# hasnainfarid/Custom_Gymnasium_Environments

Measured on AMD Instinct MI355X. Metric: env steps/sec (whole node) at 1M parallel envs; achieved HBM GB/s vs peak, higher is better.
Workload: dtype i8; 1 GPU; snake_1m: SnakeEnv 10x10, 1,048,576 parallel envs per GPU, random actions, fused auto-reset; envs_per_gpu=1048576, autoreset=SameStep, parallelism=env-sharded x1, no data-path collective

## Files before the change

custom_gymnasium_environments_amd/csrc/snake.hip:

```cpp
#include <cstdlib>
#include <cstring>
#include <vector>

#include "cge_device.hpp"
#include "cge_host.hpp"
#include "snake_place.hpp"

#ifndef CGE_SNAKE_FINCOPY
#define CGE_SNAKE_FINCOPY 1
#endif
namespace cge {
namespace snake {

constexpr int bitlen(int n) {
    int k = 0;
    while (n) { ++k; n >>= 1; }
    return k;
}

enum : uint32_t { F_NEEDS_RESET = 1u, F_BOARD_FULL = 2u, F_FOOD_VALID = 4u };

template <int G>
struct Lay {
    static constexpr int CELLS = G * G;
    static constexpr int OCCW = (CELLS + 31) / 32;
    static constexpr int SRW = (2 * (CELLS - 1) + 31) / 32;
    static constexpr bool TIGHT = (G == 10);
    static constexpr int HOT_SH = 15;
    static constexpr int HOT_DIRS = (2 * 32 - HOT_SH) / 2, COLD0_DIRS = 64;
    static constexpr int NW = TIGHT ? 12 : OCCW + SRW + 4;
    static constexpr int COLS = (NW + 3) / 4;
    static constexpr bool PACKED = CELLS % 4 == 0;
    static constexpr int OBS_DW = (CELLS + 3) / 4;
    static constexpr int KBITS = bitlen(G);
    static constexpr int BLOCK = (CELLS <= 144) ? 256 : 64;
    static_assert(G >= 4 && G <= 30, "center start needs G >= 4 (and a 10x10-style 3 cell margin is not assumed); 64 rows of G*G bytes + the digit rings fit 64 KB of LDS up to 30");
    static constexpr int MAX_STEPS_LIMIT = TIGHT ? 4095 : 65535;
    static constexpr uint32_t MAX_EPISODES = TIGHT ? 0xFFFFu : 0xFFFFFFFFu;
    static_assert(CELLS <= 1023, "cell index is packed in 10 bits");
    static_assert(!TIGHT || (SRW == 7 && OCCW == 4), "hot / cold split below is written for 10x10");
};

__host__ __device__ __forceinline__ int dir_delta(uint32_t d, int g) { return d == 0 ? -g : d == 1 ? 1 : d == 2 ? g : -1; }

template <int G>
struct Env {
    using L = Lay<G>;
    uint32_t occ[L::OCCW];
    uint32_t sr[L::SRW];
    uint32_t head, tail, len, food, dir, steps, score, flags, episodes, mt_pos, mt_pretw, dq_left;

    __device__ __forceinline__ void load(const uint4 *__restrict__ state, int64_t n, int64_t i) {
        uint32_t raw[L::COLS * 4];
        if constexpr (L::TIGHT) {
            const uint4 h = state[i];
            raw[0] = h.x; raw[1] = h.y; raw[2] = h.z; raw[3] = h.w;
            const uint32_t moves = ((h.x >> 7) & 127u) - 1u;
            uint4 c0 = make_uint4(0, 0, 0, 0), c1 = make_uint4(0, 0, 0, 0);
            if (moves > (uint32_t)L::HOT_DIRS) c0 = state[n + i];
            if (moves > (uint32_t)(L::HOT_DIRS + L::COLD0_DIRS)) c1 = state[2 * n + i];
            raw[4] = c0.x; raw[5] = c0.y; raw[6] = c0.z; raw[7] = c0.w;
            raw[8] = c1.x; raw[9] = c1.y; raw[10] = c1.z; raw[11] = c1.w;
        } else {
#pragma unroll
            for (int c = 0; c < L::COLS; ++c) {
                uint4 v = state[(int64_t)c * n + i];
                raw[4 * c] = v.x; raw[4 * c + 1] = v.y; raw[4 * c + 2] = v.z; raw[4 * c + 3] = v.w;
            }
        }
        unpack(raw);
    }
    __device__ __forceinline__ void store(uint4 *__restrict__ state, int64_t n, int64_t i) const {
        uint32_t raw[L::COLS * 4];
        pack(raw);
        if constexpr (L::TIGHT) {
            state[i] = make_uint4(raw[0], raw[1], raw[2], raw[3]);
            if (len - 1u > (uint32_t)L::HOT_DIRS) state[n + i] = make_uint4(raw[4], raw[5], raw[6], raw[7]);
            if (len - 1u > (uint32_t)(L::HOT_DIRS + L::COLD0_DIRS)) state[2 * n + i] = make_uint4(raw[8], raw[9], raw[10], raw[11]);
        } else {
#pragma unroll
            for (int c = 0; c < L::COLS; ++c)
                state[(int64_t)c * n + i] = make_uint4(raw[4 * c], raw[4 * c + 1], raw[4 * c + 2], raw[4 * c + 3]);
        }
    }
    __host__ __device__ __forceinline__ void unpack(const uint32_t *raw) {
        if constexpr (L::TIGHT) {
            const uint32_t w0 = raw[0], w1 = raw[1], w2 = raw[2];
            head = w0 & 127u; len = (w0 >> 7) & 127u; food = (w0 >> 14) & 127u; dir = (w0 >> 21) & 3u; flags = (w0 >> 23) & 7u;
            score = (w0 >> 26) | (((w1 >> 23) & 1u) << 6);
            steps = w1 & 0xFFFu; mt_pos = (w1 >> 12) & 1023u; mt_pretw = (w1 & (1u << 22)) ? (uint32_t)MT_N : 0u;
            episodes = (w1 >> 24) | ((w2 & 0xFFu) << 8);
            dq_left = (w2 >> 8) & 127u;
#pragma unroll
            for (int k = 0; k < L::SRW; ++k) sr[k] = (raw[2 + k] >> L::HOT_SH) | (raw[3 + k] << (32 - L::HOT_SH));
            mask_history();
            rebuild_occupancy();
        } else {
#pragma unroll
            for (int k = 0; k < L::OCCW; ++k) occ[k] = raw[k];
#pragma unroll
            for (int k = 0; k < L::SRW; ++k) sr[k] = raw[L::OCCW + k];
            const uint32_t m0 = raw[L::OCCW + L::SRW], m1 = raw[L::OCCW + L::SRW + 1], m3 = raw[L::OCCW + L::SRW + 3];
            head = m0 & 1023u; tail = (m0 >> 10) & 1023u; food = (m0 >> 20) & 1023u; dir = m0 >> 30;
            steps = m1 & 0xffffu; score = (m1 >> 16) & 1023u; flags = m1 >> 26;
            episodes = raw[L::OCCW + L::SRW + 2];
            mt_pos = m3 & 1023u; mt_pretw = (m3 & 1024u) ? (uint32_t)MT_N : 0u; len = (m3 >> 11) & 1023u; dq_left = (m3 >> 24) & 127u;
        }
    }
    __host__ __device__ __forceinline__ void pack(uint32_t *raw) const {
        if constexpr (L::TIGHT) {
            const uint32_t ep = episodes < L::MAX_EPISODES ? episodes : L::MAX_EPISODES;
            raw[0] = head | (len << 7) | (food << 14) | (dir << 21) | (flags << 23) | ((score & 63u) << 26);
            raw[1] = steps | (mt_pos << 12) | (mt_pretw ? (1u << 22) : 0u) | (((score >> 6) & 1u) << 23) | ((ep & 0xFFu) << 24);
            raw[2] = (ep >> 8) | (dq_left << 8) | (sr[0] << L::HOT_SH);
#pragma unroll
            for (int k = 1; k < L::SRW; ++k) raw[2 + k] = (sr[k - 1] >> (32 - L::HOT_SH)) | (sr[k] << L::HOT_SH);
            raw[2 + L::SRW] = sr[L::SRW - 1] >> (32 - L::HOT_SH);
#pragma unroll
            for (int k = 3 + L::SRW; k < 12; ++k) raw[k] = 0;
        } else {
#pragma unroll
            for (int k = 0; k < L::OCCW; ++k) raw[k] = occ[k];
#pragma unroll
            for (int k = 0; k < L::SRW; ++k) raw[L::OCCW + k] = sr[k];
            raw[L::OCCW + L::SRW] = head | (tail << 10) | (food << 20) | (dir << 30);
            raw[L::OCCW + L::SRW + 1] = steps | (score << 16) | (flags << 26);
            raw[L::OCCW + L::SRW + 2] = episodes;
            raw[L::OCCW + L::SRW + 3] = mt_pos | (mt_pretw ? 1024u : 0u) | (len << 11) | (dq_left << 24);
#pragma unroll
            for (int k = L::NW; k < L::COLS * 4; ++k) raw[k] = 0;
        }
    }
    __host__ __device__ __forceinline__ void mask_history() {
        const uint32_t bits = len == 0u ? 0u : 2u * (len - 1u);
#pragma unroll
        for (int k = 0; k < L::SRW; ++k) {
            const uint32_t lo = 32u * k;
            sr[k] = bits >= lo + 32u ? sr[k] : (bits > lo ? (sr[k] & ((1u << (bits - lo)) - 1u)) : 0u);
        }
    }
    __host__ __device__ __forceinline__ void rebuild_occupancy() {
#pragma unroll
        for (int k = 0; k < L::OCCW; ++k) occ[k] = 0;
        uint32_t cell = head;
        or_word(occ, cell >> 5, 1u << (cell & 31u));
        const uint32_t moves = len == 0u ? 0u : (len <= (uint32_t)L::CELLS ? len - 1u : (uint32_t)L::CELLS - 1u);
        uint64_t q = (uint64_t)sr[0] | ((uint64_t)sr[1] << 32);
        const uint32_t n1 = moves < 32u ? moves : 32u;
        for (uint32_t k = 0; k < n1; ++k) {
            cell = (uint32_t)((int)cell - dir_delta((uint32_t)q & 3u, G));
            q >>= 2;
            or_word(occ, cell >> 5, 1u << (cell & 31u));
        }
        for (uint32_t k = 32u; k < moves; ++k) {
            const uint32_t d = (sel(sr, k >> 4) >> ((k & 15u) * 2u)) & 3u;
            cell = (uint32_t)((int)cell - dir_delta(d, G));
            or_word(occ, cell >> 5, 1u << (cell & 31u));
        }
        tail = cell;
    }

    __host__ __device__ __forceinline__ uint32_t occupied(uint32_t cell) const {
        if constexpr (L::OCCW == 4) {
            const uint64_t lo = (uint64_t)occ[0] | ((uint64_t)occ[1] << 32), hi = (uint64_t)occ[2] | ((uint64_t)occ[3] << 32);
            return (uint32_t)(((cell < 64u ? lo : hi) >> (cell & 63u)) & 1ull);
        } else {
            return (sel(occ, cell >> 5) >> (cell & 31u)) & 1u;
        }
    }
    __host__ __device__ __forceinline__ uint32_t length() const { return len; }

    __device__ __forceinline__ bool can_place_food() {
        if (len >= (uint32_t)L::CELLS) {
            flags = (flags | F_BOARD_FULL) & ~F_FOOD_VALID;
            return false;
        }
        return true;
    }

    __device__ __forceinline__ void reset_body() {
#pragma unroll
        for (int k = 0; k < L::OCCW; ++k) occ[k] = 0;
#pragma unroll
        for (int k = 0; k < L::SRW; ++k) sr[k] = 0;
        constexpr uint32_t center = (G / 2) * G + (G / 2);
        head = tail = center;
        len = 1;
        occ[center >> 5] |= 1u << (center & 31u);
        dir = 1;
        score = 0;
        steps = 0;
        flags &= ~F_NEEDS_RESET;
    }

    __device__ __forceinline__ bool move(uint32_t action, uint32_t max_steps, float &reward, bool &ate, bool short_wave) {
        ate = false;
        const int d = (int)action - (int)dir;
        if (d != 2 && d != -2) dir = action;
        const uint32_t hr = head / G, hc = head - hr * G;
        int nr = (int)hr, nc = (int)hc;
        if (dir == 0) nr -= 1; else if (dir == 1) nc += 1; else if (dir == 2) nr += 1; else nc -= 1;
        const bool wall = (unsigned)nr >= (unsigned)G || (unsigned)nc >= (unsigned)G;
        const uint32_t ncell = wall ? head : (uint32_t)(nr * G + nc);
        if (wall || occupied(ncell)) {
            reward = -10.0f;
            return true;
        }
        if (!short_wave) {
#pragma unroll
            for (int k = L::SRW - 1; k > 0; --k) sr[k] = (sr[k] << 2) | (sr[k - 1] >> 30);
        }
        sr[0] = (sr[0] << 2) | dir;
        or_word(occ, ncell >> 5, 1u << (ncell & 31u));
        head = ncell;
        reward = 0.0f;
        if ((flags & F_FOOD_VALID) && ncell == food) {
            score += 1;
            len += 1;
            reward = 10.0f;
            ate = true;
        } else {
            const uint32_t p = 2u * (len - 1u);
            uint32_t td;
            if (short_wave) {
                td = (sr[0] >> p) & 3u;
                sr[0] &= ~(3u << p);
            } else {
                td = (sel(sr, p >> 5) >> (p & 31u)) & 3u;
                andnot_word(sr, p >> 5, 3u << (p & 31u));
            }
            andnot_word(occ, tail >> 5, 1u << (tail & 31u));
            tail = (uint32_t)((int)tail + dir_delta(td, G));
        }
        steps += 1;
        return steps >= max_steps;
    }

    __device__ __forceinline__ void write_obs_body(uint32_t *row) const {
#pragma unroll
        for (int j = 0; j < L::OBS_DW; ++j) {
            const uint32_t b = (occ[(4 * j) >> 5] >> ((4 * j) & 31)) & 0xFu;
            row[j] = (b * 0x00204081u) & 0x01010101u;
        }
    }
    __device__ __forceinline__ void write_obs_food(uint32_t *row) const {
        if (flags & F_FOOD_VALID) reinterpret_cast<int8_t *>(row)[food] = 2;
    }
};

struct Params {
    uint4 *state;
    uint4 *dq;
    uint32_t *mt;
    int64_t n, env0;
    const int32_t *actions;
    const uint8_t *mask;
    int8_t *obs;
    float *reward;
    uint8_t *terminated, *truncated;
    int8_t *final_obs;
    FinalSeg fin;
    int32_t mode, max_steps, k_steps;
    uint32_t dq_topup;
    uint64_t a_seed;
    int64_t t0, obs_step_stride;
    float *reward_sum;
    int32_t *done_count;
    double *ep_ret;
    int32_t *ep_len;
    unsigned long long *err_count;
};

__device__ __forceinline__ uint32_t shfl_u32(uint32_t v, uint32_t src) { return (uint32_t)__shfl((int)v, (int)src, 64); }

template <int G>
struct DigitQ {
    static constexpr int DB = Lay<G>::KBITS <= 4 ? 4 : 8;
    static constexpr int PER = 32 / DB;
    static constexpr int SLOTS = 64;
    static constexpr int QDW = SLOTS / PER;
    static constexpr int COLS = QDW / 4;
    static constexpr int QROW = QDW + 1;
    static constexpr uint32_t DMASK = (1u << DB) - 1u;
    static constexpr uint32_t ALL_COLS = (1u << COLS) - 1u;
};

template <int G>
struct DqCtx {
    uint32_t *wave_q;
    uint32_t stride;
    uint32_t *blk;
    uint4 *dq;
    int64_t n, i;
    uint32_t loaded;
    bool dirty;

    __device__ __forceinline__ uint32_t *my_row() const { return wave_q + (threadIdx.x & 63u) * stride; }
    __device__ __forceinline__ void issue_all(uint4 (&v)[DigitQ<G>::COLS]) const {
#pragma unroll
        for (int c = 0; c < DigitQ<G>::COLS; ++c) v[c] = dq[(int64_t)c * n + i];
    }
    __device__ __forceinline__ void park_all(const uint4 (&v)[DigitQ<G>::COLS]) {
        uint32_t *row = my_row();
#pragma unroll
        for (int c = 0; c < DigitQ<G>::COLS; ++c) { row[4 * c] = v[c].x; row[4 * c + 1] = v[c].y; row[4 * c + 2] = v[c].z; row[4 * c + 3] = v[c].w; }
        loaded = DigitQ<G>::ALL_COLS;
    }
    __device__ __forceinline__ void load_pair(bool want, uint32_t c0, uint32_t c1) {
        if (want && ((~loaded >> c0) & 1u || (~loaded >> c1) & 1u)) {
            uint32_t *row = my_row();
            const uint4 v0 = dq[(int64_t)c0 * n + i], v1 = dq[(int64_t)c1 * n + i];
            row[4 * c0] = v0.x; row[4 * c0 + 1] = v0.y; row[4 * c0 + 2] = v0.z; row[4 * c0 + 3] = v0.w;
            row[4 * c1] = v1.x; row[4 * c1 + 1] = v1.y; row[4 * c1 + 2] = v1.z; row[4 * c1 + 3] = v1.w;
            loaded |= (1u << c0) | (1u << c1);
        }
    }
    __device__ __forceinline__ void write_back() {
        using Q = DigitQ<G>;
        if (!dirty) return;
        const uint32_t *row = my_row();
#pragma unroll
        for (int c = 0; c < Q::COLS; ++c) dq[(int64_t)c * n + i] = make_uint4(row[4 * c], row[4 * c + 1], row[4 * c + 2], row[4 * c + 3]);
        dirty = false;
    }
};

template <int G, int RG = 2>
__device__ __forceinline__ void dq_refill(Env<G> &e, DqCtx<G> &q, unsigned long long want) {
    using L = Lay<G>;
    using Q = DigitQ<G>;
    const uint32_t lane = threadIdx.x & 63u;
    const uint32_t plo = (uint32_t)reinterpret_cast<uintptr_t>(q.blk), phi = (uint32_t)(reinterpret_cast<uintptr_t>(q.blk) >> 32);
#pragma unroll 1
    while (want) {
        int r[RG];
        bool has[RG];
        uint32_t pos[RG], pretw[RG], left[RG], fill[RG], k[RG], a[RG], b[RG], c[RG];
        uint32_t *ob[RG];
#pragma unroll
        for (int g = 0; g < RG; ++g) {
            has[g] = want != 0ull;
            r[g] = has[g] ? (int)__builtin_ctzll(want) : r[0];
            want = has[g] ? (want & (want - 1ull)) : 0ull;
            uint32_t p = lane_u32(e.mt_pos, r[g]) & 1023u, lf = lane_u32(e.dq_left, r[g]) & 127u, pt = lane_u32(e.mt_pretw, r[g]);
            p = p < (uint32_t)MT_N ? p : (uint32_t)MT_N;
            lf = lf < (uint32_t)Q::SLOTS ? lf : (uint32_t)Q::SLOTS;
            if (p == (uint32_t)MT_N && lf == 0u) { p = 0u; pt = 0u; }
            const uint32_t room = (uint32_t)Q::SLOTS - lf, rest = (uint32_t)MT_N - p;
            pos[g] = p; pretw[g] = pt; left[g] = lf; fill[g] = room < rest ? room : rest;
            const uint32_t j = (lane - p) & 63u;
            const uint32_t kk = j < fill[g] ? p + j : (p < (uint32_t)MT_N ? p : 0u);
            const uint32_t km = kk + MT_M >= (uint32_t)MT_N ? kk + MT_M - MT_N : kk + MT_M;
            k[g] = kk;
            ob[g] = lane_ptr(plo, phi, r[g]);
            a[g] = ob[g][kk]; b[g] = ob[g][kk + 1]; c[g] = ob[g][km];
        }
#pragma unroll
        for (int g = 0; g < RG; ++g) {
            if (!has[g]) continue;
            const bool active = ((lane - pos[g]) & 63u) < fill[g];
            const bool ready = k[g] < pretw[g];
            const uint32_t y = ready ? a[g] : mt_twist(a[g], b[g], c[g]);
            if (active && !ready) mt_store(ob[g], k[g], y);
            const uint32_t sh = (lane % Q::PER) * Q::DB;
            uint32_t x = active ? (mt_temper(y) >> (32 - L::KBITS)) << sh : 0u;
            uint32_t m = active ? Q::DMASK << sh : 0u;
            x |= shfl_u32(x, lane ^ 1u); m |= shfl_u32(m, lane ^ 1u);
            x |= shfl_u32(x, lane ^ 2u); m |= shfl_u32(m, lane ^ 2u);
            if (Q::PER == 8) { x |= shfl_u32(x, lane ^ 4u); m |= shfl_u32(m, lane ^ 4u); }
            uint32_t *row = q.wave_q + (uint32_t)r[g] * q.stride;
            if (lane % Q::PER == 0u && m) row[lane / Q::PER] = (row[lane / Q::PER] & ~m) | x;
            if (lane == (uint32_t)r[g]) {
                e.mt_pos = pos[g] + fill[g];
                e.mt_pretw = pretw[g];
                e.dq_left = left[g] + fill[g];
                q.dirty = true;
                q.loaded = Q::ALL_COLS;
            }
        }
    }
}

template <int G>
__device__ __forceinline__ bool dq_can_fill(const Env<G> &e) {
    return e.dq_left < (uint32_t)DigitQ<G>::SLOTS && !(e.mt_pos >= (uint32_t)MT_N && e.dq_left > 0u);
}

template <int G, bool FETCH>
__device__ __forceinline__ void dq_place_food(Env<G> &e, DqCtx<G> &q, bool need) {
    using L = Lay<G>;
    using Q = DigitQ<G>;
    const uint32_t *myq = q.my_row();
    bool pending = need;
    uint32_t phase = 0, row = 0;
#pragma unroll 1
    while (__ballot(pending)) {
        if (FETCH) {
            const uint32_t head = (e.mt_pos - e.dq_left) & 63u, d0 = head / Q::PER, d1 = (d0 + 1u) & (uint32_t)(Q::QDW - 1);
            q.load_pair(pending && e.dq_left != 0u, d0 >> 2, d1 >> 2);
        }
        const unsigned long long dry = __ballot(pending && e.dq_left < (uint32_t)Q::PER && dq_can_fill<G>(e));
// ... 280 lines not shown
        const uint32_t fin_deferred = (FIN && MODE == CGE_AUTORESET_SAME_STEP) ? fin_used + (uint32_t)__popcll(__ballot(term && !(tf & T_DEFERRED))) : 0u;
        bool want = need_food;
#pragma unroll 1
        for (int round = 0; round < 2; ++round) {
            dq_place_food<G, false>(e, q, want);
            if (round == 1 || __ballot(tf & T_DEFERRED) == 0ull) break;
            want = (tf & T_DEFERRED) && finish_deferred<G, FIN>(e, p, i, nullptr, t, fin_deferred);
            if (tf & T_DEFERRED) { was_reset = true; need_food = want; }
        }
        if (FIN && MODE == CGE_AUTORESET_SAME_STEP) fin_used += (uint32_t)__popcll(__ballot(term));
        if (row) {
            unsigned long long rm = __ballot(was_reset);
            while (rm) {
                const uint32_t rl = (uint32_t)__ffsll((long long)rm) - 1u;
                rm &= rm - 1ull;
                if (lane < (uint32_t)L::OBS_DW) wave_rows[rl * L::OBS_DW + lane] = 0u;
                if (L::OBS_DW > 64) for (uint32_t q2 = lane + 64u; q2 < (uint32_t)L::OBS_DW; q2 += 64u) wave_rows[rl * L::OBS_DW + q2] = 0u;
            }
            if (live_lane) {
                if (was_reset) rowb[e.head] = 1;
                else if (e.head != old_head) { rowb[e.head] = 1; if (e.tail != old_tail) rowb[old_tail] = 0; }
                if (need_food) e.write_obs_food(row);
            }
            int8_t *dst_t = p.obs + (int64_t)t * p.obs_step_stride + wfirst * L::CELLS;
            if constexpr (L::PACKED) store_wave_rows<64 * L::CELLS>(wave_rows, dst_t, (uint32_t)(wlive * L::CELLS), lane);
            else store_rows_realign<L::CELLS, L::OBS_DW>(wave_rows, dst_t, (uint32_t)wlive, lane, 64u);
        }
        if (live_lane) {
            rsum += r;
            dcount += term ? 1 : 0;
            if (p.reward) p.reward[(int64_t)t * p.n + i] = r;
            if (p.terminated) p.terminated[(int64_t)t * p.n + i] = term ? 1 : 0;
        }
    }
    if (live_lane) {
        e.store(p.state, p.n, i);
        q.write_back();
        if (p.reward_sum) p.reward_sum[i] = rsum;
        if (p.done_count) p.done_count[i] = dcount;
        if (FIN && p.fin.count && (threadIdx.x & 63u) == 0u) p.fin.count[wfirst >> 6] = (int32_t)fin_used;
    }
}

template <int G>
__global__ __launch_bounds__(Lay<G>::BLOCK) void reset_kernel(Params p) {
    using L = Lay<G>;
    using Q = DigitQ<G>;
    __shared__ uint4 tile4[(L::BLOCK * L::OBS_DW + 3) / 4];
    __shared__ uint32_t qmem[L::BLOCK * Q::QROW];
    uint32_t *tile = reinterpret_cast<uint32_t *>(tile4);
    const int64_t first = (int64_t)blockIdx.x * L::BLOCK;
    const int64_t i = first + threadIdx.x;
    const bool live_lane = i < p.n;
    const int64_t li = live_lane ? i : first;
    Env<G> e;
    e.load(p.state, p.n, li);
    uint32_t *row = p.obs ? tile + threadIdx.x * L::OBS_DW : nullptr;
    const bool doit = live_lane && (!p.mask || p.mask[i]);
    bool need_food = false;
    if (doit) {
        e.reset_body();
        need_food = e.can_place_food();
    }
    if (row) e.write_obs_body(row);
    DqCtx<G> q{qmem + (threadIdx.x & ~63u) * Q::QROW, (uint32_t)Q::QROW, p.mt + li * MT_STRIDE, p.dq, p.n, li, 0u, false};
    dq_place_food<G, true>(e, q, need_food);
    if (row) e.write_obs_food(row);
    if (doit) { e.store(p.state, p.n, i); q.write_back(); }
    if (p.obs) {
        lds_barrier();
        const int64_t live = p.n - first < L::BLOCK ? p.n - first : L::BLOCK;
        if constexpr (L::PACKED) store_tile<L::BLOCK>(tile, p.obs + first * L::CELLS, (uint32_t)(live * L::CELLS));
        else store_rows_realign<L::CELLS, L::OBS_DW>(tile, p.obs + first * L::CELLS, (uint32_t)live, threadIdx.x, L::BLOCK);
    }
}

template <int G>
__global__ __launch_bounds__(256) void rewind_kernel(uint4 *__restrict__ state, int64_t n) {
    const int64_t i = (int64_t)blockIdx.x * 256 + threadIdx.x;
    if (i >= n) return;
    Env<G> e;
    e.load(state, n, i);
    e.mt_pos = 0;
    e.mt_pretw = 0;
    e.dq_left = 0;
    e.store(state, n, i);
}

template <int G>
__global__ __launch_bounds__(256) void info_kernel(const uint4 *__restrict__ state, int64_t n, int field, int32_t *__restrict__ out) {
    const int64_t i = (int64_t)blockIdx.x * 256 + threadIdx.x;
    if (i >= n) return;
    Env<G> e;
    e.load(state, n, i);
    int32_t v = 0;
    const bool fv = e.flags & F_FOOD_VALID;
    switch (field) {
        case CGE_SNAKE_INFO_SCORE: v = (int32_t)e.score; break;
        case CGE_SNAKE_INFO_LENGTH: v = (int32_t)e.length(); break;
        case CGE_SNAKE_INFO_STEPS: v = (int32_t)e.steps; break;
        case CGE_SNAKE_INFO_DIRECTION: v = (int32_t)e.dir; break;
        case CGE_SNAKE_INFO_FOOD_R: v = fv ? (int32_t)(e.food / G) : -1; break;
        case CGE_SNAKE_INFO_FOOD_C: v = fv ? (int32_t)(e.food % G) : -1; break;
        case CGE_SNAKE_INFO_BOARD_FULL: v = (e.flags & F_BOARD_FULL) ? 1 : 0; break;
        case CGE_SNAKE_INFO_EPISODES: v = (int32_t)e.episodes; break;
        case CGE_SNAKE_INFO_HEAD_R: v = (int32_t)(e.head / G); break;
        case CGE_SNAKE_INFO_HEAD_C: v = (int32_t)(e.head % G); break;
        case CGE_SNAKE_INFO_NEEDS_RESET: v = (e.flags & F_NEEDS_RESET) ? 1 : 0; break;
    }
    out[i] = v;
}

template <int G>
__global__ __launch_bounds__(256) void render_kernel(const uint4 *__restrict__ state, int64_t n, uint32_t *__restrict__ out) {
    using L = Lay<G>;
    constexpr int64_t ROWB = (int64_t)L::CELLS * 3;
    const int64_t total = n * ROWB, ndw = (total + 3) / 4;
    const int64_t gid = (int64_t)blockIdx.x * 256 + threadIdx.x;
    if (gid >= ndw) return;
    int64_t i = (4 * gid) / ROWB;
    uint32_t within = (uint32_t)(4 * gid - i * ROWB);
    Env<G> e;
    e.load(state, n, i < n ? i : n - 1);
    uint32_t w = 0, nb = 0;
#pragma unroll
    for (uint32_t b = 0; b < 4; ++b) {
        if (4 * gid + b >= total) break;
        if (within == (uint32_t)ROWB) { within = 0; ++i; e.load(state, n, i); }
        const uint32_t cell = within / 3u, ch = within - 3u * cell;
        const bool fv = e.flags & F_FOOD_VALID;
        uint32_t v = 0;
        if (fv && cell == e.food) v = ch == 0u ? 255u : 0u;
        else if (e.occupied(cell)) v = ch == 1u ? 255u : 0u;
        w |= v << (8u * b);
        ++within; ++nb;
    }
    if (nb == 4) out[gid] = w;
    else for (uint32_t b = 0; b < nb; ++b) reinterpret_cast<uint8_t *>(out)[4 * gid + b] = (uint8_t)(w >> (8u * b));
}

struct Ops {
    int cells, cols, block, nw, max_steps_limit;
    void (*rewind)(uint4 *, int64_t, hipStream_t);
    int dq_cols;
    void (*step)(const Params &, hipStream_t, std::string *);
    void (*rollout)(const Params &, hipStream_t, std::string *);
    void (*reset)(const Params &, hipStream_t);
    void (*info)(const uint4 *, int64_t, int, int32_t *, hipStream_t);
    void (*render)(const uint4 *, int64_t, uint32_t *, hipStream_t);
    void (*decode)(const uint32_t *raw, int32_t *hdr, uint16_t *body, uint32_t *mt_pos, uint32_t *mt_pretw, uint32_t *dq_left);
    bool (*encode)(const int32_t *hdr, const uint16_t *body, uint32_t mt_pos, uint32_t mt_pretw, uint32_t *raw);
};

template <int G>
void decode_env(const uint32_t *raw, int32_t *hdr, uint16_t *body, uint32_t *mt_pos, uint32_t *mt_pretw, uint32_t *dq_left) {
    using L = Lay<G>;
    Env<G> e;
    e.unpack(raw);
    *mt_pos = e.mt_pos;
    *mt_pretw = e.mt_pretw;
    *dq_left = e.dq_left;
    const int len = (int)e.length();
    const bool fv = e.flags & F_FOOD_VALID;
    hdr[0] = len; hdr[1] = (int32_t)e.dir;
    hdr[2] = fv ? (int32_t)(e.food / G) : -1; hdr[3] = fv ? (int32_t)(e.food % G) : -1;
    hdr[4] = (int32_t)e.score; hdr[5] = (int32_t)e.steps; hdr[6] = (e.flags & F_NEEDS_RESET) ? 1 : 0;
    uint32_t c = e.head;
    for (int k = 0; k < L::CELLS; ++k) {
        body[k] = k < len ? (uint16_t)c : 0xFFFF;
        if (k + 1 < len) c = (uint32_t)((int)c - dir_delta((e.sr[k >> 4] >> ((k & 15) * 2)) & 3u, G));
    }
}

template <int G>
bool encode_env(const int32_t *hdr, const uint16_t *body, uint32_t mt_pos, uint32_t mt_pretw, uint32_t *raw) {
    Env<G> e;
    memset(&e, 0, sizeof e);
    const int len = hdr[0];
    for (int k = 0; k < len; ++k) {
        if (e.occ[body[k] >> 5] & (1u << (body[k] & 31u))) return false;
        e.occ[body[k] >> 5] |= 1u << (body[k] & 31u);
    }
    for (int k = 0; k + 1 < len; ++k) {
        const int from = body[k + 1], to = body[k];
        uint32_t d;
        if (to == from - G) d = 0u;
        else if (to == from + 1 && from % G != G - 1) d = 1u;
        else if (to == from + G) d = 2u;
        else if (to == from - 1 && from % G != 0) d = 3u;
        else return false;
        e.sr[k >> 4] |= d << ((k & 15) * 2);
    }
    e.head = body[0];
    e.tail = body[len - 1];
    e.len = (uint32_t)len;
    e.dir = (uint32_t)hdr[1];
    const bool fv = hdr[2] >= 0;
    e.food = fv ? (uint32_t)(hdr[2] * G + hdr[3]) : 0u;
    e.score = (uint32_t)hdr[4];
    e.steps = (uint32_t)hdr[5];
    e.flags = (hdr[6] ? F_NEEDS_RESET : 0u) | (fv ? F_FOOD_VALID : 0u);
    e.episodes = 0;
    e.mt_pos = mt_pos; e.mt_pretw = mt_pretw;
    e.pack(raw);
    return true;
}

template <int G, int BLOCK, int MINW, int MODE>
void launch_mode(const Params &p, bool rollout, hipStream_t s, std::string *name) {
    const dim3 grid((unsigned)((p.n + BLOCK - 1) / BLOCK)), block(BLOCK);
    char buf[96];
    if (!rollout) {
        hipLaunchKernelGGL((step_kernel<G, BLOCK, MINW, MODE>), grid, block, 0, s, p);
        snprintf(buf, sizeof buf, "cge::snake::step_kernel<%d, %d, %d, %d>", G, BLOCK, MINW, MODE);
    } else {
        const bool fin = p.fin.rows != nullptr;
        if (p.actions) { if (fin) hipLaunchKernelGGL((rollout_kernel<G, BLOCK, MINW, MODE, true, true>), grid, block, 0, s, p);
                         else hipLaunchKernelGGL((rollout_kernel<G, BLOCK, MINW, MODE, true, false>), grid, block, 0, s, p); }
        else { if (fin) hipLaunchKernelGGL((rollout_kernel<G, BLOCK, MINW, MODE, false, true>), grid, block, 0, s, p);
               else hipLaunchKernelGGL((rollout_kernel<G, BLOCK, MINW, MODE, false, false>), grid, block, 0, s, p); }
        snprintf(buf, sizeof buf, "cge::snake::rollout_kernel<%d, %d, %d, %d, %s, %s>", G, BLOCK, MINW, MODE, p.actions ? "true" : "false", fin ? "true" : "false");
    }
    if (name) *name = buf;
}
template <int G, int BLOCK, int MINW>
void launch_any(const Params &p, bool rollout, hipStream_t s, std::string *name) {
    if (p.mode == CGE_AUTORESET_SAME_STEP) launch_mode<G, BLOCK, MINW, CGE_AUTORESET_SAME_STEP>(p, rollout, s, name);
    else if (p.mode == CGE_AUTORESET_NEXT_STEP) launch_mode<G, BLOCK, MINW, CGE_AUTORESET_NEXT_STEP>(p, rollout, s, name);
    else launch_mode<G, BLOCK, MINW, CGE_AUTORESET_DISABLED>(p, rollout, s, name);
}

constexpr int MAX_RAW = 4 * Lay<30>::COLS;

template <int G>
Ops make_ops() {
    using L = Lay<G>;
    Ops o;
    o.cells = L::CELLS; o.cols = L::COLS; o.block = L::BLOCK; o.nw = L::NW; o.max_steps_limit = L::MAX_STEPS_LIMIT;
    o.dq_cols = DigitQ<G>::COLS;
    o.rewind = [](uint4 *st, int64_t n, hipStream_t s) {
        hipLaunchKernelGGL(rewind_kernel<G>, dim3((unsigned)((n + 255) / 256)), dim3(256), 0, s, st, n);
    };
    o.step = [](const Params &p, hipStream_t s, std::string *name) { launch_any<G, L::BLOCK, 1>(p, false, s, name); };
    o.rollout = [](const Params &p, hipStream_t s, std::string *name) { launch_any<G, L::BLOCK, 1>(p, true, s, name); };
    o.reset = [](const Params &p, hipStream_t s) {
        hipLaunchKernelGGL(reset_kernel<G>, dim3((unsigned)((p.n + L::BLOCK - 1) / L::BLOCK)), dim3(L::BLOCK), 0, s, p);
    };
    o.info = [](const uint4 *st, int64_t n, int field, int32_t *out, hipStream_t s) {
        hipLaunchKernelGGL(info_kernel<G>, dim3((unsigned)((n + 255) / 256)), dim3(256), 0, s, st, n, field, out);
    };
    o.render = [](const uint4 *st, int64_t n, uint32_t *out, hipStream_t s) {
        const int64_t total = (n * (int64_t)L::CELLS * 3 + 3) / 4;
        hipLaunchKernelGGL(render_kernel<G>, dim3((unsigned)((total + 255) / 256)), dim3(256), 0, s, st, n, out);
    };
    o.decode = decode_env<G>;
    o.encode = encode_env<G>;
    return o;
}

static bool ops_for(int grid, Ops &o) {
    switch (grid) {
#define CGE_GRID(G_) case G_: o = make_ops<G_>(); return true;
        CGE_GRID(4) CGE_GRID(5) CGE_GRID(6) CGE_GRID(7) CGE_GRID(8) CGE_GRID(9) CGE_GRID(10) CGE_GRID(11) CGE_GRID(12) CGE_GRID(13)
        CGE_GRID(14) CGE_GRID(15) CGE_GRID(16) CGE_GRID(17) CGE_GRID(18) CGE_GRID(19) CGE_GRID(20) CGE_GRID(21) CGE_GRID(22)
        CGE_GRID(23) CGE_GRID(24) CGE_GRID(25) CGE_GRID(26) CGE_GRID(27) CGE_GRID(28) CGE_GRID(29) CGE_GRID(30)
#undef CGE_GRID
    }
    return false;
}

}
}

using namespace cge;

struct cge_snake : HandleBase {
    cge_snake_config cfg{};
    snake::Ops ops{};
    uint4 *state = nullptr;
    uint4 *dq = nullptr;
    uint32_t *mt = nullptr;
    unsigned long long *err = nullptr;

    snake::Params params() const {
        snake::Params p{};
        p.state = state; p.dq = dq; p.mt = mt; p.n = n; p.env0 = env0;
        p.mode = cfg.autoreset_mode; p.max_steps = cfg.max_steps; p.err_count = err;
        p.ep_ret = ep_ret; p.ep_len = ep_len;
        return p;
    }
    static int check(const cge_snake_config &c) {
        if (bad_autoreset_mode(c.autoreset_mode) || c.max_steps < 0 || c.max_steps > 65535) return CGE_ERR_INVALID_ARG;
        snake::Ops o;
        return snake::ops_for(c.grid_size, o) && (c.max_steps ? c.max_steps : 1000) <= o.max_steps_limit ? CGE_OK : CGE_ERR_UNSUPPORTED;
    }
    hipError_t init() {
        if (cfg.max_steps == 0) cfg.max_steps = 1000;
        snake::ops_for(cfg.grid_size, ops);
        CGE_HIP(alloc(state, (size_t)ops.cols * n * sizeof(uint4), true, false));
        CGE_HIP(alloc(mt, (size_t)n * MT_STRIDE * sizeof(uint32_t), false, false));
        CGE_HIP(alloc(dq, (size_t)ops.dq_cols * n * sizeof(uint4), true, false));
        CGE_HIP(alloc(err, sizeof(unsigned long long), true, false));
        CGE_HIP(launch_mt_seed(mt, MT_STRIDE, n, nullptr, 0, env0, 0, nullptr));
        ops.reset(params(), nullptr);
        return hipGetLastError();
    }

    static constexpr const char *abi = "cge_snake";
    enum { A_STATE, A_MT };
    size_t record_bytes() const { return (8 * 4 + (size_t)MT_N * 4 + (size_t)ops.cells * 2 + 3) & ~(size_t)3; }
    std::vector<RecordArray> record_arrays() const {
        return {{state, sizeof(uint4), ops.cols, false, true}, {mt, sizeof(uint32_t), MT_STRIDE, true, true}};
    }
    const char *check_record(const uint8_t *p) const {
        const int32_t *hdr = (const int32_t *)p;
        const uint16_t *body = (const uint16_t *)(p + 32 + MT_N * 4);
        const int cells = ops.cells, G = cfg.grid_size;
        if (hdr[0] < 1 || hdr[0] > cells || hdr[1] < 0 || hdr[1] > 3 || hdr[7] < 0 || hdr[7] > MT_N) return "malformed record";
        const bool no_food = hdr[2] == -1 && hdr[3] == -1;
        if ((!no_food && (hdr[2] < 0 || hdr[2] >= G || hdr[3] < 0 || hdr[3] >= G)) || hdr[4] < 0 || hdr[4] > cells || hdr[5] < 0 ||
            hdr[5] > ops.max_steps_limit || (hdr[6] != 0 && hdr[6] != 1))
            return "food / score / steps / needs_reset out of range";
        for (int k = 0; k < hdr[0]; ++k)
            if (body[k] >= cells) return "body cell out of range";
        uint32_t raw[snake::MAX_RAW];
        return ops.encode(hdr, body, 0u, 0u, raw) ? nullptr : "the body is not a path of unit moves";
    }
    int to_record(const RecordStage &st, int64_t j, uint8_t *p, const char **why) const {
        uint32_t raw[snake::MAX_RAW];
        for (int c = 0; c < ops.cols; ++c) memcpy(raw + 4 * c, st.at<uint4>(A_STATE, j, c), 16);
        int32_t *hdr = (int32_t *)p;
        uint32_t pos = 0, pretw = 0, left = 0;
        ops.decode(raw, hdr, (uint16_t *)(p + 32 + MT_N * 4), &pos, &pretw, &left);
        if (left > pos) { *why = "corrupted digit-ring cursor"; return CGE_ERR_INVALID_ARG; }
        int32_t idx = 0;
        mt_export_cpython(st.at<uint32_t>(A_MT, j), pos, pretw, (uint32_t *)(p + 32), &idx);
        hdr[7] = idx - (int32_t)left;
        return CGE_OK;
    }
    void from_record(const uint8_t *p, RecordStage &st, int64_t j) const {
        const int32_t *hdr = (const int32_t *)p;
        uint32_t raw[snake::MAX_RAW], pos, pretw;
        mt_import_cpython((const uint32_t *)(p + 32), hdr[7], st.at<uint32_t>(A_MT, j), &pos, &pretw);
        ops.encode(hdr, (const uint16_t *)(p + 32 + MT_N * 4), pos, pretw, raw);
        for (int c = 0; c < ops.cols; ++c) memcpy(st.at<uint4>(A_STATE, j, c), raw + 4 * c, 16);
    }
};

extern "C" {

const char *cge_version(void) { return "cge_amd 0.1 (gfx950)"; }

uint32_t cge_hash_action(uint64_t a_seed, uint64_t env, uint64_t t, uint32_t n, uint32_t j) {
    return hash_action_from_key(hash_env_key(a_seed, env), t, n, j);
}

CGE_DEFINE_LIFECYCLE(snake)

int cge_snake_seed(cge_snake *h, const uint64_t *seeds, uint64_t base_seed, void *stream) {
    if (!h) return CGE_ERR_INVALID_ARG;
    DeviceGuard g(h->device);
    CGE_TRY(h, launch_mt_seed(h->mt, MT_STRIDE, h->n, seeds, base_seed, h->env0, 0, as_stream(stream)));
    h->ops.rewind(h->state, h->n, as_stream(stream));
    return launched(h);
}

int cge_snake_reset(cge_snake *h, const uint8_t *mask, int8_t *obs_out, void *stream) {
    if (!h) return CGE_ERR_INVALID_ARG;
    DeviceGuard g(h->device);
    snake::Params p = h->params();
    p.mask = mask;
    p.obs = obs_out;
    h->ops.reset(p, as_stream(stream));
    return launched(h);
}

int cge_snake_step(cge_snake *h, const int32_t *actions, int8_t *obs_out, float *reward_out, uint8_t *terminated_out,
                   uint8_t *truncated_out, int8_t *final_obs_out, void *stream) {
    snake::Params p;
    if (int st = step_params(h, p, actions && obs_out && reward_out && terminated_out, "cge_snake_step: null actions/obs/reward/terminated pointer",
                             obs_out, reward_out, terminated_out, truncated_out, final_obs_out)) return st;
    DeviceGuard g(h->device);
    p.actions = actions;
    h->ops.step(p, as_stream(stream), &h->last_kernel);
    return launched(h);
}

int cge_snake_rollout(cge_snake *h, int32_t k_steps, const int32_t *actions, uint64_t action_seed, int64_t t0,
                      int8_t *obs_out, int64_t obs_step_stride, float *reward_traj_out, uint8_t *terminated_traj_out,
                      float *reward_sum_out, int32_t *done_count_out, void *stream) {
    if (!h) return CGE_ERR_INVALID_ARG;
    snake::Params p;
    const bool aligned = !((obs_step_stride & 3) && h->ops.cells % 4 == 0);
    const int st = rollout_params(h, p, aligned, h->n * h->ops.cells, "cge_snake_rollout: bad k_steps / obs_step_stride", k_steps, action_seed, t0,
                                  obs_out, obs_step_stride, reward_traj_out, terminated_traj_out, reward_sum_out, done_count_out);
    if (st != CGE_OK || k_steps == 0) return st;
    DeviceGuard g(h->device);
    p.actions = actions;
    p.dq_topup = 12u;
#ifdef CGE_SNAKE_TOPUP_ENV
    if (const char *ev = getenv("CGE_SNAKE_TOPUP")) p.dq_topup = (uint32_t)atoi(ev);
#endif
    h->ops.rollout(p, as_stream(stream), &h->last_kernel);
    return launched(h);
}

CGE_DEFINE_FINAL_OBS(snake, int8_t, 64)

int cge_snake_info(cge_snake *h, int32_t field_id, int32_t *out, void *stream) {
    if (!h) return CGE_ERR_INVALID_ARG;
    if (!out || field_id < 0 || field_id > CGE_SNAKE_INFO_NEEDS_RESET)
        return h->fail(CGE_ERR_INVALID_ARG, "cge_snake_info: bad field id / null out");
    DeviceGuard g(h->device);
    h->ops.info(h->state, h->n, field_id, out, as_stream(stream));
    return launched(h);
}

int cge_snake_render_rgb(cge_snake *h, uint8_t *rgb_out, void *stream) {
    if (!h) return CGE_ERR_INVALID_ARG;
    if (!rgb_out || (reinterpret_cast<uintptr_t>(rgb_out) & 3u)) return h->fail(CGE_ERR_INVALID_ARG, "cge_snake_render_rgb: null or unaligned rgb_out");
    DeviceGuard g(h->device);
    h->ops.render(h->state, h->n, reinterpret_cast<uint32_t *>(rgb_out), as_stream(stream));
    return launched(h);
}

CGE_DEFINE_RECORDS(snake)

CGE_DEFINE_ERROR_COUNT(snake)

}
```

Baseline: 50.28 billion env-steps/s.

## Make snake move branchless with packed direction tables and cached head row/col

```diff
diff --git a/custom_gymnasium_environments_amd/csrc/snake.hip b/custom_gymnasium_environments_amd/csrc/snake.hip
--- a/custom_gymnasium_environments_amd/csrc/snake.hip
+++ b/custom_gymnasium_environments_amd/csrc/snake.hip
@@ -41,7 +41,18 @@
     static_assert(!TIGHT || (SRW == 7 && OCCW == 4), "hot / cold split below is written for 10x10");
 };
 
-__host__ __device__ __forceinline__ int dir_delta(uint32_t d, int g) { return d == 0 ? -g : d == 1 ? 1 : d == 2 ? g : -1; }
+__host__ __device__ __forceinline__ int table_field(uint32_t tab, uint32_t pos, uint32_t width) {
+#if defined(__HIP_DEVICE_COMPILE__)
+    return __builtin_amdgcn_sbfe((int)tab, pos, width);
+#else
+    return (int32_t)(tab << (32u - width - pos)) >> (32u - width);
+#endif
+}
+__host__ __device__ __forceinline__ int dir_delta(uint32_t d, int g) {
+    return table_field(((uint32_t)(-g) & 0xFFu) | (1u << 8) | ((uint32_t)g << 16) | (0xFFu << 24), 8u * d, 8u);
+}
+__host__ __device__ __forceinline__ int dir_drow(uint32_t d) { return table_field(0x13u, 2u * d, 2u); }
+__host__ __device__ __forceinline__ int dir_dcol(uint32_t d) { return table_field(0xC4u, 2u * d, 2u); }
 
 template <int G>
 struct Env {
@@ -49,6 +60,7 @@
     uint32_t occ[L::OCCW];
     uint32_t sr[L::SRW];
     uint32_t head, tail, len, food, dir, steps, score, flags, episodes, mt_pos, mt_pretw, dq_left;
+    uint32_t hr, hc;
 
     __device__ __forceinline__ void load(const uint4 *__restrict__ state, int64_t n, int64_t i) {
         uint32_t raw[L::COLS * 4];
@@ -69,7 +81,9 @@
             }
         }
         unpack(raw);
-    }
+        locate_head();
+    }
+    __host__ __device__ __forceinline__ void locate_head() { hr = head / (uint32_t)G; hc = head - hr * (uint32_t)G; }
     __device__ __forceinline__ void store(uint4 *__restrict__ state, int64_t n, int64_t i) const {
         uint32_t raw[L::COLS * 4];
         pack(raw);
@@ -143,19 +157,19 @@
 #pragma unroll
         for (int k = 0; k < L::OCCW; ++k) occ[k] = 0;
         uint32_t cell = head;
-        or_word(occ, cell >> 5, 1u << (cell & 31u));
+        occ_set(cell);
         const uint32_t moves = len == 0u ? 0u : (len <= (uint32_t)L::CELLS ? len - 1u : (uint32_t)L::CELLS - 1u);
         uint64_t q = (uint64_t)sr[0] | ((uint64_t)sr[1] << 32);
         const uint32_t n1 = moves < 32u ? moves : 32u;
         for (uint32_t k = 0; k < n1; ++k) {
             cell = (uint32_t)((int)cell - dir_delta((uint32_t)q & 3u, G));
             q >>= 2;
-            or_word(occ, cell >> 5, 1u << (cell & 31u));
+            occ_set(cell);
         }
         for (uint32_t k = 32u; k < moves; ++k) {
             const uint32_t d = (sel(sr, k >> 4) >> ((k & 15u) * 2u)) & 3u;
             cell = (uint32_t)((int)cell - dir_delta(d, G));
-            or_word(occ, cell >> 5, 1u << (cell & 31u));
+            occ_set(cell);
         }
         tail = cell;
     }
@@ -168,6 +182,26 @@
             return (sel(occ, cell >> 5) >> (cell & 31u)) & 1u;
         }
     }
+    __host__ __device__ __forceinline__ void occ_set(uint32_t cell) {
+        if constexpr (L::OCCW == 4) {
+            const uint64_t m = 1ull << (cell & 63u);
+            const uint32_t ml = (uint32_t)m, mh = (uint32_t)(m >> 32);
+            const bool up = (cell & 64u) != 0u;
+            occ[0] |= up ? 0u : ml; occ[1] |= up ? 0u : mh; occ[2] |= up ? ml : 0u; occ[3] |= up ? mh : 0u;
+        } else {
+            or_word(occ, cell >> 5, 1u << (cell & 31u));
+        }
+    }
+    __host__ __device__ __forceinline__ void occ_clear_if(uint32_t cell, bool on) {
+        if constexpr (L::OCCW == 4) {
+            const uint64_t m = 1ull << (cell & 63u);
+            const uint32_t ml = (uint32_t)m, mh = (uint32_t)(m >> 32);
+            const bool lo = on && (cell & 64u) == 0u, up = on && (cell & 64u) != 0u;
+            occ[0] &= ~(lo ? ml : 0u); occ[1] &= ~(lo ? mh : 0u); occ[2] &= ~(up ? ml : 0u); occ[3] &= ~(up ? mh : 0u);
+        } else {
+            andnot_word(occ, cell >> 5, on ? 1u << (cell & 31u) : 0u);
+        }
+    }
     __host__ __device__ __forceinline__ uint32_t length() const { return len; }
 
     __device__ __forceinline__ bool can_place_food() {
@@ -178,13 +212,14 @@
         return true;
     }
 
-    __device__ __forceinline__ void reset_body() {
+    __host__ __device__ __forceinline__ void reset_body() {
 #pragma unroll
         for (int k = 0; k < L::OCCW; ++k) occ[k] = 0;
 #pragma unroll
         for (int k = 0; k < L::SRW; ++k) sr[k] = 0;
         constexpr uint32_t center = (G / 2) * G + (G / 2);
         head = tail = center;
+        hr = hc = G / 2;
         len = 1;
         occ[center >> 5] |= 1u << (center & 31u);
         dir = 1;
@@ -193,47 +228,39 @@
         flags &= ~F_NEEDS_RESET;
     }
 
-    __device__ __forceinline__ bool move(uint32_t action, uint32_t max_steps, float &reward, bool &ate, bool short_wave) {
+    __host__ __device__ __forceinline__ bool move(uint32_t action, uint32_t max_steps, float &reward, bool &ate, bool short_wave) {
         ate = false;
-        const int d = (int)action - (int)dir;
-        if (d != 2 && d != -2) dir = action;
-        const uint32_t hr = head / G, hc = head - hr * G;
-        int nr = (int)hr, nc = (int)hc;
-        if (dir == 0) nr -= 1; else if (dir == 1) nc += 1; else if (dir == 2) nr += 1; else nc -= 1;
-        const bool wall = (unsigned)nr >= (unsigned)G || (unsigned)nc >= (unsigned)G;
-        const uint32_t ncell = wall ? head : (uint32_t)(nr * G + nc);
-        if (wall || occupied(ncell)) {
-            reward = -10.0f;
-            return true;
-        }
-        if (!short_wave) {
+        dir = ((action ^ dir) != 2u) ? action : dir;
+        const uint32_t nr = hr + (uint32_t)dir_drow(dir), nc = hc + (uint32_t)dir_dcol(dir);
+        const uint32_t ncell = nr * (uint32_t)G + nc;
+        const bool wall = (nr > nc ? nr : nc) >= (uint32_t)G;
+        const bool ok = !(wall | (occupied(ncell) != 0u));
+        const bool eat = ok && (flags & F_FOOD_VALID) && ncell == food;
+        const uint32_t p = 2u * (len - 1u);
+        uint32_t td = 0u;
+        if (__builtin_expect(short_wave, true)) {
+            const uint32_t s0 = (sr[0] << 2) | dir;
+            td = (s0 >> p) & 3u;
+            sr[0] = ok ? s0 & ~(eat ? 0u : 3u << p) : sr[0];
+        } else if (ok) {
 #pragma unroll
             for (int k = L::SRW - 1; k > 0; --k) sr[k] = (sr[k] << 2) | (sr[k - 1] >> 30);
-        }
-        sr[0] = (sr[0] << 2) | dir;
-        or_word(occ, ncell >> 5, 1u << (ncell & 31u));
-        head = ncell;
-        reward = 0.0f;
-        if ((flags & F_FOOD_VALID) && ncell == food) {
-            score += 1;
-            len += 1;
-            reward = 10.0f;
-            ate = true;
-        } else {
-            const uint32_t p = 2u * (len - 1u);
-            uint32_t td;
-            if (short_wave) {
-                td = (sr[0] >> p) & 3u;
-                sr[0] &= ~(3u << p);
-            } else {
-                td = (sel(sr, p >> 5) >> (p & 31u)) & 3u;
-                andnot_word(sr, p >> 5, 3u << (p & 31u));
-            }
-            andnot_word(occ, tail >> 5, 1u << (tail & 31u));
-            tail = (uint32_t)((int)tail + dir_delta(td, G));
-        }
-        steps += 1;
-        return steps >= max_steps;
+            sr[0] = (sr[0] << 2) | dir;
+            td = (sel(sr, p >> 5) >> (p & 31u)) & 3u;
+            andnot_word(sr, p >> 5, eat ? 0u : 3u << (p & 31u));
+        }
+        reward = ok ? (eat ? 10.0f : 0.0f) : -10.0f;
+        ate = eat;
+        if (ok) {
+            occ_set(ncell);
+            head = ncell; hr = nr; hc = nc;
+            occ_clear_if(tail, !eat);
+            tail = (uint32_t)((int)tail + (eat ? 0 : dir_delta(td, G)));
+            score += eat ? 1u : 0u;
+            len += eat ? 1u : 0u;
+            steps += 1;
+        }
+        return !ok || steps >= max_steps;
     }
 
     __device__ __forceinline__ void write_obs_body(uint32_t *row) const {
@@ -247,6 +274,67 @@
         if (flags & F_FOOD_VALID) reinterpret_cast<int8_t *>(row)[food] = 2;
     }
 };
+
+template <int G>
+void decode_env(const uint32_t *raw, int32_t *hdr, uint16_t *body, uint32_t *mt_pos, uint32_t *mt_pretw, uint32_t *dq_left) {
+    using L = Lay<G>;
+    Env<G> e;
+    e.unpack(raw);
+    *mt_pos = e.mt_pos;
+    *mt_pretw = e.mt_pretw;
+    *dq_left = e.dq_left;
+    const int len = (int)e.length();
+    const bool fv = e.flags & F_FOOD_VALID;
+    hdr[0] = len; hdr[1] = (int32_t)e.dir;
+    hdr[2] = fv ? (int32_t)(e.food / G) : -1; hdr[3] = fv ? (int32_t)(e.food % G) : -1;
+    hdr[4] = (int32_t)e.score; hdr[5] = (int32_t)e.steps; hdr[6] = (e.flags & F_NEEDS_RESET) ? 1 : 0;
+    uint32_t c = e.head;
+    for (int k = 0; k < L::CELLS; ++k) {
+        body[k] = k < len ? (uint16_t)c : 0xFFFF;
+        if (k + 1 < len) c = (uint32_t)((int)c - dir_delta((e.sr[k >> 4] >> ((k & 15) * 2)) & 3u, G));
+    }
+}
+
+template <int G>
+bool encode_env(const int32_t *hdr, const uint16_t *body, uint32_t mt_pos, uint32_t mt_pretw, uint32_t *raw) {
+    Env<G> e;
+    memset(&e, 0, sizeof e);
+    const int len = hdr[0];
+    for (int k = 0; k < len; ++k) {
+        if (e.occ[body[k] >> 5] & (1u << (body[k] & 31u))) return false;
+        e.occ[body[k] >> 5] |= 1u << (body[k] & 31u);
+    }
+    for (int k = 0; k + 1 < len; ++k) {
+        const int from = body[k + 1], to = body[k];
+        uint32_t d;
+        if (to == from - G) d = 0u;
+        else if (to == from + 1 && from % G != G - 1) d = 1u;
+        else if (to == from + G) d = 2u;
+        else if (to == from - 1 && from % G != 0) d = 3u;
+        else return false;
+        e.sr[k >> 4] |= d << ((k & 15) * 2);
+    }
+    e.head = body[0];
+    e.tail = body[len - 1];
+    e.len = (uint32_t)len;
+    e.dir = (uint32_t)hdr[1];
+    const bool fv = hdr[2] >= 0;
+    e.food = fv ? (uint32_t)(hdr[2] * G + hdr[3]) : 0u;
+    e.score = (uint32_t)hdr[4];
+    e.steps = (uint32_t)hdr[5];
+    e.flags = (hdr[6] ? F_NEEDS_RESET : 0u) | (fv ? F_FOOD_VALID : 0u);
+    e.episodes = 0;
+    e.mt_pos = mt_pos; e.mt_pretw = mt_pretw;
+    e.pack(raw);
+    return true;
+}
+
+}
+}
+
+#ifndef CGE_SNAKE_ENV_ONLY
+namespace cge {
+namespace snake {
 
 struct Params {
     uint4 *state;
@@ -833,60 +921,6 @@
     bool (*encode)(const int32_t *hdr, const uint16_t *body, uint32_t mt_pos, uint32_t mt_pretw, uint32_t *raw);
 };
 
-template <int G>
-void decode_env(const uint32_t *raw, int32_t *hdr, uint16_t *body, uint32_t *mt_pos, uint32_t *mt_pretw, uint32_t *dq_left) {
-    using L = Lay<G>;
-    Env<G> e;
-    e.unpack(raw);
-    *mt_pos = e.mt_pos;
-    *mt_pretw = e.mt_pretw;
-    *dq_left = e.dq_left;
-    const int len = (int)e.length();
-    const bool fv = e.flags & F_FOOD_VALID;
-    hdr[0] = len; hdr[1] = (int32_t)e.dir;
-    hdr[2] = fv ? (int32_t)(e.food / G) : -1; hdr[3] = fv ? (int32_t)(e.food % G) : -1;
-    hdr[4] = (int32_t)e.score; hdr[5] = (int32_t)e.steps; hdr[6] = (e.flags & F_NEEDS_RESET) ? 1 : 0;
-    uint32_t c = e.head;
-    for (int k = 0; k < L::CELLS; ++k) {
-        body[k] = k < len ? (uint16_t)c : 0xFFFF;
-        if (k + 1 < len) c = (uint32_t)((int)c - dir_delta((e.sr[k >> 4] >> ((k & 15) * 2)) & 3u, G));
-    }
-}
-
-template <int G>
-bool encode_env(const int32_t *hdr, const uint16_t *body, uint32_t mt_pos, uint32_t mt_pretw, uint32_t *raw) {
-    Env<G> e;
-    memset(&e, 0, sizeof e);
-    const int len = hdr[0];
-    for (int k = 0; k < len; ++k) {
-        if (e.occ[body[k] >> 5] & (1u << (body[k] & 31u))) return false;
-        e.occ[body[k] >> 5] |= 1u << (body[k] & 31u);
-    }
-    for (int k = 0; k + 1 < len; ++k) {
-        const int from = body[k + 1], to = body[k];
-        uint32_t d;
-        if (to == from - G) d = 0u;
-        else if (to == from + 1 && from % G != G - 1) d = 1u;
-        else if (to == from + G) d = 2u;
-        else if (to == from - 1 && from % G != 0) d = 3u;
-        else return false;
-        e.sr[k >> 4] |= d << ((k & 15) * 2);
-    }
-    e.head = body[0];
-    e.tail = body[len - 1];
-    e.len = (uint32_t)len;
-    e.dir = (uint32_t)hdr[1];
-    const bool fv = hdr[2] >= 0;
-    e.food = fv ? (uint32_t)(hdr[2] * G + hdr[3]) : 0u;
-    e.score = (uint32_t)hdr[4];
-    e.steps = (uint32_t)hdr[5];
-    e.flags = (hdr[6] ? F_NEEDS_RESET : 0u) | (fv ? F_FOOD_VALID : 0u);
-    e.episodes = 0;
-    e.mt_pos = mt_pos; e.mt_pretw = mt_pretw;
-    e.pack(raw);
-    return true;
-}
-
 template <int G, int BLOCK, int MINW, int MODE>
 void launch_mode(const Params &p, bool rollout, hipStream_t s, std::string *name) {
     const dim3 grid((unsigned)((p.n + BLOCK - 1) / BLOCK)), block(BLOCK);
@@ -1110,3 +1144,4 @@
 CGE_DEFINE_ERROR_COUNT(snake)
 
 }
+#endif
```

Result: no change. 50.71 billion env-steps/s (median of 6 runs) (+0.9%).
